# Lance0218/Pytorch-DistributedDataParallel-Training-Tricks

Measured on AMD Instinct MI355X. Metric: images/sec, higher is better.
Workload: dtype bf16; 1 GPU; model=Toy_Net, dataset=MNIST(synthetic), global_batch=1024, per_gpu_batch=1024, parallelism=dp1, optimizer=FusedSGD(momentum=0.9,nesterov)+Lookahead(k=10,a=0.5)

## Files before the change

### ddp_tricks_amd/ops/hip/bindings.cpp

```cpp
#include <torch/extension.h>

void multi_tensor_unscale(std::vector<at::Tensor> grads, at::Tensor found_inf,
                          double inv_scale,
                          c10::optional<at::Tensor> partials);
void multi_tensor_sqsum(std::vector<at::Tensor> tensors, at::Tensor partials);
void norm_finalize(at::Tensor partials, long n, double max_norm,
                   c10::optional<at::Tensor> found_inf, at::Tensor out,
                   c10::optional<at::Tensor> stats);
void multi_tensor_scale(std::vector<at::Tensor> tensors, at::Tensor coef,
                        c10::optional<at::Tensor> found_inf);
long mt_chunk_elems();
void fused_sgd(std::vector<at::Tensor> params, std::vector<at::Tensor> grads,
               std::vector<at::Tensor> bufs, double lr, double momentum,
               double wd, double nesterov, c10::optional<at::Tensor> found_inf,
               c10::optional<at::Tensor> grad_scale);
void fused_lookahead(std::vector<at::Tensor> fast, std::vector<at::Tensor> slow,
                     double alpha, c10::optional<at::Tensor> found_inf);
at::Tensor cast_to_bf16(at::Tensor x);
at::Tensor pad8_channels(at::Tensor x);
at::Tensor nhwc_flatten(at::Tensor x);
at::Tensor nhwc_unflatten(at::Tensor dy, long C, long H, long W);
std::vector<at::Tensor> pack_conv_weight(at::Tensor w, bool pad8,
                                         bool want_wt2);

std::vector<at::Tensor> ce_fwd(at::Tensor logits, at::Tensor target);
at::Tensor ce_bwd(at::Tensor logits, at::Tensor target, at::Tensor lse,
                  at::Tensor dloss);
at::Tensor argmax_correct(at::Tensor logits, at::Tensor target);

std::vector<at::Tensor> maxpool2x2_fwd(at::Tensor x);
at::Tensor maxpool2x2_bwd(at::Tensor dy, at::Tensor idx, long H, long W);
std::vector<at::Tensor> maxpool_fwd(at::Tensor x, long ks, long st, long pad);
at::Tensor maxpool_bwd(at::Tensor dy, at::Tensor idx, long H, long W,
                       long ks, long st, long pad);
at::Tensor global_avgpool_fwd(at::Tensor x);
at::Tensor global_avgpool_bwd(at::Tensor dy, long H, long W);

std::vector<at::Tensor> bn_fwd_train(at::Tensor x, at::Tensor gamma,
                                     at::Tensor beta, at::Tensor running_mean,
                                     at::Tensor running_var, double momentum,
                                     double eps, bool fuse_relu,
                                     c10::optional<at::Tensor> residual,
                                     c10::optional<at::Tensor> pre_stats);
at::Tensor bn_fwd_eval(at::Tensor x, at::Tensor gamma, at::Tensor beta,
                       at::Tensor running_mean, at::Tensor running_var,
                       double eps, bool fuse_relu,
                       c10::optional<at::Tensor> residual);
std::vector<at::Tensor> bn_fwd_eval_mask(at::Tensor x, at::Tensor gamma,
                                         at::Tensor beta,
                                         at::Tensor running_mean,
                                         at::Tensor running_var, double eps,
                                         bool fuse_relu,
                                         c10::optional<at::Tensor> residual);
std::vector<at::Tensor> bn_bwd(at::Tensor x, at::Tensor dy, at::Tensor gamma,
                               at::Tensor save_mean, at::Tensor save_invstd,
                               at::Tensor mask, bool fuse_relu,
                               bool want_dresid,
                               c10::optional<at::Tensor> pre_slab,
                               bool eval_stats);
std::vector<at::Tensor> bn_fwd_train_pool2(at::Tensor x, at::Tensor gamma,
                                           at::Tensor beta,
                                           at::Tensor running_mean,
                                           at::Tensor running_var,
                                           double momentum, double eps,
                                           c10::optional<at::Tensor> pre_stats);
std::vector<at::Tensor> bn_bwd_pool2(at::Tensor x, at::Tensor dy_pooled,
                                     at::Tensor gamma, at::Tensor save_mean,
                                     at::Tensor save_invstd, at::Tensor code);

at::Tensor gemm_tn(at::Tensor A, at::Tensor B, c10::optional<at::Tensor> bias,
                   bool out_f32);
at::Tensor transpose_bf16(at::Tensor x);
at::Tensor col_sum(at::Tensor x);
at::Tensor linear_fwd(at::Tensor x, at::Tensor w, c10::optional<at::Tensor> bias);
at::Tensor linear_dgrad(at::Tensor dy, at::Tensor w);
at::Tensor linear_wgrad(at::Tensor dy, at::Tensor x);

at::Tensor conv2d_fwd(at::Tensor x, at::Tensor w, c10::optional<at::Tensor> bias,
                      long stride, long pad);
std::vector<at::Tensor> conv2d_fwd_stats(at::Tensor x, at::Tensor w,
                                         c10::optional<at::Tensor> bias,
                                         long stride, long pad);
at::Tensor conv2d_dgrad(at::Tensor dy, at::Tensor wt2, long N, long C, long H,
                        long W, long R, long S, long stride, long pad,
                        c10::optional<at::Tensor> addend);
std::vector<at::Tensor> conv2d_dgrad_bn(at::Tensor dy, at::Tensor wt2,
                                        long N, long C, long H, long W,
                                        long R, long S, long pad,
                                        at::Tensor bn_x, at::Tensor bn_mask,
                                        at::Tensor bn_mean,
                                        at::Tensor bn_invstd);
at::Tensor conv2d_wgrad(at::Tensor dy, at::Tensor x, long R, long S,
                        long stride, long pad);
std::vector<at::Tensor> conv2d_wgrad_bias(at::Tensor dy, at::Tensor x,
                                          long R, long S, long stride,
                                          long pad);
std::tuple<std::string, long, bool> conv2d_wgrad_plan(
    long N, long C, long H, long W, long Ko, long R, long S, long stride,
    long pad, bool want_bias);

std::vector<at::Tensor> batch_gather_aug(at::Tensor store, at::Tensor labels,
                                         at::Tensor index, at::Tensor lut,
                                         long pad, bool hflip, long seed,
                                         long epoch);

void register_comm(py::module_& m);

PYBIND11_MODULE(TORCH_EXTENSION_NAME, m) {
    register_comm(m);
    m.def("multi_tensor_unscale", &multi_tensor_unscale,
          "fused unscale + inf check over grad tensors; with partials also "
          "the per-chunk sums of squares of the unscaled values",
          py::arg("grads"), py::arg("found_inf"), py::arg("inv_scale"),
          py::arg("partials") = c10::nullopt);
    m.def("multi_tensor_sqsum", &multi_tensor_sqsum,
          "per-chunk sums of squares (read-only)",
          py::arg("tensors"), py::arg("partials"));
    m.def("norm_finalize", &norm_finalize,
          "partials -> out = {2-norm, clip coefficient} (+ telemetry)",
          py::arg("partials"), py::arg("n"), py::arg("max_norm"),
          py::arg("found_inf"), py::arg("out"), py::arg("stats"));
    m.def("multi_tensor_scale", &multi_tensor_scale,
          "tensors *= coef[0] in place (device coefficient)",
          py::arg("tensors"), py::arg("coef"),
          py::arg("found_inf") = c10::nullopt);
    m.attr("MT_CHUNK") = mt_chunk_elems();
    m.def("fused_sgd", &fused_sgd, "fused nesterov-momentum SGD step",
          py::arg("params"), py::arg("grads"), py::arg("bufs"), py::arg("lr"),
          py::arg("momentum"), py::arg("wd"), py::arg("nesterov"),
          py::arg("found_inf") = c10::nullopt,
          py::arg("grad_scale") = c10::nullopt);
    m.def("fused_lookahead", &fused_lookahead, "fused Lookahead interpolation",
          py::arg("fast"), py::arg("slow"), py::arg("alpha"),
          py::arg("found_inf") = c10::nullopt);
    m.def("cast_to_bf16", &cast_to_bf16);
    m.def("pad8_channels", &pad8_channels);
    m.def("nhwc_flatten", &nhwc_flatten);
    m.def("nhwc_unflatten", &nhwc_unflatten);
    m.def("pack_conv_weight", &pack_conv_weight, py::arg("w"),
          py::arg("pad8") = false, py::arg("want_wt2") = true);
    m.def("ce_fwd", &ce_fwd);
    m.def("ce_bwd", &ce_bwd);
    m.def("argmax_correct", &argmax_correct);
    m.def("maxpool2x2_fwd", &maxpool2x2_fwd);
    m.def("maxpool2x2_bwd", &maxpool2x2_bwd);
    m.def("maxpool_fwd", &maxpool_fwd);
    m.def("maxpool_bwd", &maxpool_bwd);
    m.def("global_avgpool_fwd", &global_avgpool_fwd);
    m.def("global_avgpool_bwd", &global_avgpool_bwd);
    m.def("bn_fwd_train", &bn_fwd_train,
          py::arg("x"), py::arg("gamma"), py::arg("beta"),
          py::arg("running_mean"), py::arg("running_var"), py::arg("momentum"),
          py::arg("eps"), py::arg("fuse_relu") = false,
          py::arg("residual") = c10::nullopt,
          py::arg("pre_stats") = c10::nullopt);
    m.def("bn_fwd_eval", &bn_fwd_eval,
          py::arg("x"), py::arg("gamma"), py::arg("beta"),
          py::arg("running_mean"), py::arg("running_var"), py::arg("eps"),
          py::arg("fuse_relu") = false, py::arg("residual") = c10::nullopt);
    m.def("bn_bwd", &bn_bwd,
          py::arg("x"), py::arg("dy"), py::arg("gamma"), py::arg("save_mean"),
          py::arg("save_invstd"), py::arg("mask"), py::arg("fuse_relu") = false,
          py::arg("want_dresid") = false, py::arg("pre_slab") = c10::nullopt,
          py::arg("eval_stats") = false);
    m.def("bn_fwd_eval_mask", &bn_fwd_eval_mask,
          py::arg("x"), py::arg("gamma"), py::arg("beta"),
          py::arg("running_mean"), py::arg("running_var"), py::arg("eps"),
          py::arg("fuse_relu") = false, py::arg("residual") = c10::nullopt);
    m.def("bn_fwd_train_pool2", &bn_fwd_train_pool2,
          "BN(train) + ReLU + 2x2/s2 max-pool in one apply pass",
          py::arg("x"), py::arg("gamma"), py::arg("beta"),
          py::arg("running_mean"), py::arg("running_var"), py::arg("momentum"),
          py::arg("eps"), py::arg("pre_stats") = c10::nullopt);
    m.def("bn_bwd_pool2", &bn_bwd_pool2,
          py::arg("x"), py::arg("dy_pooled"), py::arg("gamma"),
          py::arg("save_mean"), py::arg("save_invstd"), py::arg("code"));
    m.def("gemm_tn", &gemm_tn, py::arg("A"), py::arg("B"),
          py::arg("bias") = c10::nullopt, py::arg("out_f32") = false);
    m.def("transpose_bf16", &transpose_bf16);
    m.def("col_sum", &col_sum);
    m.def("linear_fwd", &linear_fwd, py::arg("x"), py::arg("w"),
          py::arg("bias") = c10::nullopt);
    m.def("linear_dgrad", &linear_dgrad);
    m.def("linear_wgrad", &linear_wgrad);
    m.def("conv2d_fwd", &conv2d_fwd, py::arg("x"), py::arg("w"),
          py::arg("bias") = c10::nullopt, py::arg("stride") = 1,
          py::arg("pad") = 0);
    m.def("conv2d_fwd_stats", &conv2d_fwd_stats, py::arg("x"), py::arg("w"),
          py::arg("bias") = c10::nullopt, py::arg("stride") = 1,
          py::arg("pad") = 0);
    m.def("conv2d_dgrad", &conv2d_dgrad,
          py::arg("dy"), py::arg("wt2"), py::arg("N"), py::arg("C"),
          py::arg("H"), py::arg("W"), py::arg("R"), py::arg("S"),
          py::arg("stride"), py::arg("pad"),
          py::arg("addend") = c10::nullopt);
    m.def("conv2d_dgrad_bn", &conv2d_dgrad_bn);
    m.def("conv2d_wgrad", &conv2d_wgrad);
    m.def("conv2d_wgrad_bias", &conv2d_wgrad_bias);
    m.def("conv2d_wgrad_plan", &conv2d_wgrad_plan,
          "(leaf name, split, fused_bias) conv2d_wgrad[_bias] would run for "
          "this shape under this process's DDPX_WGRAD_V; launches nothing",
          py::arg("N"), py::arg("C"), py::arg("H"), py::arg("W"),
          py::arg("Ko"), py::arg("R"), py::arg("S"), py::arg("stride"),
          py::arg("pad"), py::arg("want_bias"));
    m.def("batch_gather_aug", &batch_gather_aug,
          "uint8 HWC device store -> (bf16 channels_last batch, labels): "
          "gather by index + crop/flip + LUT normalise in one launch",
          py::arg("store"), py::arg("labels"), py::arg("index"),
          py::arg("lut"), py::arg("pad"), py::arg("hflip"), py::arg("seed"),
          py::arg("epoch"));
}
```

### ddp_tricks_amd/ops/hip/conv.hip

```cpp

#include <torch/extension.h>
#include <ATen/hip/HIPContext.h>
#include <climits>
#include <string>
#include <tuple>
#include "common.h"

typedef short bf16x8_t __attribute__((ext_vector_type(8)));

constexpr int CBM = 128, CBK = 64;

struct ConvShape {
    int N, H, W, C;
    int Ko, R, S;
    int P, Q;
    int stride, pad;
    FastDiv fdQ, fdP, fdW, fdH, fdC, fdS, fdKo;
    int cls_a, cls_b, nr, ns;
    int taps_r[4], taps_s[4];
    int off_r[4], off_s[4];
    int Hfull, Wfull;
    FastDiv fdNs;
};

static inline void init_fastdiv(ConvShape& cs) {
    cs.fdQ.init(cs.Q); cs.fdP.init(cs.P); cs.fdW.init(cs.W);
    cs.fdH.init(cs.H); cs.fdC.init(cs.C); cs.fdS.init(cs.S);
    cs.fdKo.init(cs.Ko);
}


__device__ __align__(16) unsigned char g_zero16[16];

struct BnFuse {
    const bf16* x;
    const unsigned char* mask;
    const float* mean;
    const float* invstd;
    float* slab;
};

template <int MODE, int TBN, int WAVES_M, int WAVES_N, bool STRIDE1,
          int CBM_T>
__device__ __forceinline__
void conv_gemm_body(const bf16* __restrict__ Asrc,
                    const bf16* __restrict__ Bsrc,
                    const float* __restrict__ bias, bf16* __restrict__ out,
                    const ConvShape& cs, int M, int Kgemm, int Nout,
                    float* __restrict__ stats, BnFuse bn,
                    const bf16* __restrict__ addin) {
    constexpr int WM = CBM_T / WAVES_M;
    constexpr int WN = TBN / WAVES_N;
    constexpr int MI = WM / 16;
    constexpr int NI = WN / 16;
    constexpr int A_CHUNKS = CBM_T / 8;
    constexpr int B_CHUNKS = TBN / 8;
    __shared__ bf16 lds_a[1][CBM_T][CBK];
    __shared__ bf16 lds_b[1][TBN][CBK];
    const int m0 = blockIdx.x * CBM_T;
    const int n0 = blockIdx.y * TBN;
    const int tid = threadIdx.x;
    const int lane = tid & 63;
    const int wid = tid >> 6;
    const int wr = wid / WAVES_N, wc = wid % WAVES_N;

    f32x4 acc[MI][NI] = {};
    const int pl_row = lane >> 3;
    const int pl_segp = lane & 7;

    constexpr int A_PER = A_CHUNKS / 4;
    long ri_nb[A_PER];
    int ri_u[A_PER], ri_v[A_PER];
    #pragma unroll
    for (int ci = 0; ci < A_PER; ++ci) {
        const int ch = wid + ci * 4;
        const int row = ch * 8 + pl_row;
        const int gm = m0 + row;
        ri_u[ci] = INT_MIN;
        if (gm < M) {
            if (MODE == 0) {
                unsigned rem = fd_div(gm, cs.fdQ);
                int q = fd_mod(gm, cs.fdQ, rem);
                unsigned n = fd_div(rem, cs.fdP);
                int p = fd_mod(rem, cs.fdP, n);
                ri_nb[ci] = (long)n * cs.H;
                ri_u[ci] = p * cs.stride - cs.pad;
                ri_v[ci] = q * cs.stride - cs.pad;
            } else if (MODE == 2) {
                unsigned rem = fd_div(gm, cs.fdW);
                int w1 = fd_mod(gm, cs.fdW, rem);
                unsigned n = fd_div(rem, cs.fdH);
                int h1 = fd_mod(rem, cs.fdH, n);
                ri_nb[ci] = (long)n * cs.P;
                ri_u[ci] = h1;
                ri_v[ci] = w1;
            } else {
                unsigned rem = fd_div(gm, cs.fdW);
                int wcol = fd_mod(gm, cs.fdW, rem);
                unsigned n = fd_div(rem, cs.fdH);
                int h = fd_mod(rem, cs.fdH, n);
                ri_nb[ci] = (long)n * cs.P;
                ri_u[ci] = h + cs.pad;
                ri_v[ci] = wcol + cs.pad;
            }
        }
    }

    auto issue_tile = [&](int kt, int buf) {
        #pragma unroll
        for (int ci = 0; ci < A_PER; ++ci) {
            const int ch = wid + ci * 4;
            int row = ch * 8 + pl_row;
            int seg = pl_segp ^ (row & 7);
            int gk = kt + seg * 8;
            const bf16* src = reinterpret_cast<const bf16*>(g_zero16);
            if (ri_u[ci] != INT_MIN && gk < Kgemm) {
                if (MODE == 0) {
                    unsigned rs = fd_div(gk, cs.fdC);
                    int c = fd_mod(gk, cs.fdC, rs);
                    int r = fd_div(rs, cs.fdS);
                    int sx = fd_mod(rs, cs.fdS, r);
                    int h = ri_u[ci] + r;
                    int wcol = ri_v[ci] + sx;
                    if (h >= 0 && h < cs.H && wcol >= 0 && wcol < cs.W)
                        src = &Asrc[((ri_nb[ci] + h) * cs.W + wcol) * cs.C + c];
                } else if (MODE == 2) {
                    unsigned rs2 = fd_div(gk, cs.fdKo);
                    int ko = fd_mod(gk, cs.fdKo, rs2);
                    int ti = fd_div(rs2, cs.fdNs);
                    int si = fd_mod(rs2, cs.fdNs, ti);
                    int p = ri_u[ci] + cs.off_r[ti];
                    int q = ri_v[ci] + cs.off_s[si];
                    if (p >= 0 && p < cs.P && q >= 0 && q < cs.Q)
                        src = &Asrc[((ri_nb[ci] + p) * cs.Q + q) * cs.Ko + ko];
                } else if (STRIDE1) {
                    unsigned rs = fd_div(gk, cs.fdKo);
                    int ko = fd_mod(gk, cs.fdKo, rs);
                    int r = fd_div(rs, cs.fdS);
                    int sx = fd_mod(rs, cs.fdS, r);
                    int p = ri_u[ci] - r;
                    int q = ri_v[ci] - sx;
                    if (p >= 0 && p < cs.P && q >= 0 && q < cs.Q)
                        src = &Asrc[((ri_nb[ci] + p) * cs.Q + q) * cs.Ko + ko];
                } else {
                    unsigned rs = fd_div(gk, cs.fdKo);
                    int ko = fd_mod(gk, cs.fdKo, rs);
                    int r = fd_div(rs, cs.fdS);
                    int sx = fd_mod(rs, cs.fdS, r);
                    int pn = ri_u[ci] - r;
                    int qn = ri_v[ci] - sx;
                    int p = pn / cs.stride, q = qn / cs.stride;
                    if (pn >= 0 && qn >= 0 && pn == p * cs.stride &&
                        qn == q * cs.stride && p < cs.P && q < cs.Q)
                        src = &Asrc[((ri_nb[ci] + p) * cs.Q + q) * cs.Ko + ko];
                }
            }
            __builtin_amdgcn_global_load_lds(
                (const __attribute__((address_space(1))) unsigned short*)src,
                (__attribute__((address_space(3))) unsigned short*)&lds_a[buf][ch * 8][0],
                16, 0, 0);
        }
        for (int ch = wid; ch < B_CHUNKS; ch += 4) {
            int row = ch * 8 + pl_row;
            int seg = pl_segp ^ (row & 7);
            int gn = n0 + row, gk = kt + seg * 8;
            const bf16* src = reinterpret_cast<const bf16*>(g_zero16);
            if (MODE == 2) {
                if (gn < Nout && gk < Kgemm) {
                    unsigned rs2 = fd_div(gk, cs.fdKo);
                    int ko = fd_mod(gk, cs.fdKo, rs2);
                    int ri = fd_div(rs2, cs.fdNs);
                    int si = fd_mod(rs2, cs.fdNs, ri);
                    long gk_full = ((long)cs.taps_r[ri] * cs.S
                                    + cs.taps_s[si]) * cs.Ko + ko;
                    src = &Bsrc[(long)gn * (cs.R * cs.S * cs.Ko) + gk_full];
                }
            } else if (gn < Nout && gk < Kgemm)
                src = &Bsrc[(long)gn * Kgemm + gk];
            __builtin_amdgcn_global_load_lds(
                (const __attribute__((address_space(1))) unsigned short*)src,
                (__attribute__((address_space(3))) unsigned short*)&lds_b[buf][ch * 8][0],
                16, 0, 0);
        }
    };

    constexpr int buf = 0;
    for (int kt = 0; kt < Kgemm; kt += CBK) {
        issue_tile(kt, 0);
        __syncthreads();
        #pragma unroll
        for (int ks = 0; ks < CBK; ks += 32) {
            bf16x8_t af[MI], bfr[NI];
            const int kgrp = (ks >> 3) + (lane >> 4);
            #pragma unroll
            for (int mi = 0; mi < MI; ++mi) {
                int row = wr * WM + mi * 16 + (lane & 15);
                af[mi] = *reinterpret_cast<const bf16x8_t*>(
                    &lds_a[buf][row][(kgrp ^ (row & 7)) * 8]);
            }
            #pragma unroll
            for (int ni = 0; ni < NI; ++ni) {
                int row = wc * WN + ni * 16 + (lane & 15);
                bfr[ni] = *reinterpret_cast<const bf16x8_t*>(
                    &lds_b[buf][row][(kgrp ^ (row & 7)) * 8]);
            }
            #pragma unroll
            for (int mi = 0; mi < MI; ++mi)
                #pragma unroll
                for (int ni = 0; ni < NI; ++ni)
                    acc[mi][ni] = __builtin_amdgcn_mfma_f32_16x16x32_bf16(
                        af[mi], bfr[ni], acc[mi][ni], 0, 0, 0);
        }
        __syncthreads();
    }

    float psum[NI] = {}, psq[NI] = {};
    #pragma unroll
    for (int mi = 0; mi < MI; ++mi)
        #pragma unroll
        for (int ni = 0; ni < NI; ++ni) {
            int col = n0 + wc * WN + ni * 16 + (lane & 15);
            if (col >= Nout) continue;
            float badd = bias ? bias[col] : 0.f;
            #pragma unroll
            for (int r = 0; r < 4; ++r) {
                int row = m0 + wr * WM + mi * 16 + (lane >> 4) * 4 + r;
                if (row >= M) continue;
                if (MODE == 0 && stats) {
                    float v = acc[mi][ni][r] + badd;
                    psum[ni] += v;
                    psq[ni] = fmaf(v, v, psq[ni]);
                }
                if (MODE == 2) {
                    unsigned rem = fd_div(row, cs.fdW);
                    int w1 = fd_mod(row, cs.fdW, rem);
                    unsigned n = fd_div(rem, cs.fdH);
                    int h1 = fd_mod(rem, cs.fdH, n);
                    long addr = (((long)n * cs.Hfull + cs.cls_a
                                  + (long)h1 * cs.stride) * cs.Wfull
                                 + cs.cls_b + (long)w1 * cs.stride) * Nout
                                + col;
                    out[addr] = f2bf(acc[mi][ni][r] + badd);
                }
            }
        }

    if (MODE != 2) {
        __syncthreads();
        bf16* stageA = &lds_a[0][0][0];
        bf16* stageB = &lds_b[0][0][0];
        constexpr int HALF = CBM_T * CBK;
        auto stage_at = [&](int i) -> bf16& {
            return i < HALF ? stageA[i] : stageB[i - HALF];
        };
        #pragma unroll
        for (int mi = 0; mi < MI; ++mi)
            #pragma unroll
            for (int ni = 0; ni < NI; ++ni) {
                int cl = wc * WN + ni * 16 + (lane & 15);
                float badd2 = (bias && n0 + cl < Nout) ? bias[n0 + cl] : 0.f;
                #pragma unroll
                for (int r = 0; r < 4; ++r) {
                    int rl = wr * WM + mi * 16 + (lane >> 4) * 4 + r;
                    stage_at(rl * TBN + cl) = f2bf(acc[mi][ni][r] + badd2);
                }
            }
        __syncthreads();
        constexpr int ROWS_PER_PASS = 256 / (TBN / 8);
        const int rsub = tid / (TBN / 8);
        const int csub = (tid % (TBN / 8)) * 8;
        const bool do_bn = MODE == 1 && bn.slab != nullptr;
        float bsum[8] = {}, bsx[8] = {};
        float bmean[8], binv[8];
        if (do_bn && n0 + csub < Nout) {
            #pragma unroll
            for (int j = 0; j < 8; ++j) {
                bmean[j] = bn.mean[n0 + csub + j];
                binv[j] = bn.invstd[n0 + csub + j];
            }
        }
        for (int r0_ = 0; r0_ < CBM_T; r0_ += ROWS_PER_PASS) {
            int rl = r0_ + rsub;
            long row = (long)m0 + rl;
            int col = n0 + csub;
            if (rl < CBM_T && row < M && col < Nout) {
                int i = rl * TBN + csub;
                const bf16* src16 = i < HALF ? &stageA[i] : &stageB[i - HALF];
                bf16x8_t v = *reinterpret_cast<const bf16x8_t*>(src16);
                if (MODE == 1 && addin) {
                    s16x8 a8 = *reinterpret_cast<const s16x8*>(
                        &addin[row * Nout + col]);
                    s16x8& vv = reinterpret_cast<s16x8&>(v);
                    #pragma unroll
                    for (int j = 0; j < 8; ++j)
                        vv[j] = (short)f2us(us2f((unsigned short)vv[j])
                                            + us2f((unsigned short)a8[j]));
                }
                *reinterpret_cast<bf16x8_t*>(&out[row * Nout + col]) = v;
                if (do_bn) {
                    unsigned m8 = bn.mask
                        ? bn.mask[row * (Nout >> 3) + (col >> 3)] : 0xffu;
                    s16x8 xv = *reinterpret_cast<const s16x8*>(
                        &bn.x[row * Nout + col]);
                    #pragma unroll
                    for (int j = 0; j < 8; ++j) {
                        float g = (m8 >> j) & 1u
                            ? us2f((unsigned short)((s16x8&)v)[j]) : 0.f;
                        float xh = (us2f((unsigned short)xv[j]) - bmean[j])
                                   * binv[j];
                        bsum[j] += g;
                        bsx[j] = fmaf(g, xh, bsx[j]);
                    }
                }
            }
        }
        if (do_bn) {
            __syncthreads();
            float* red = reinterpret_cast<float*>(stageA);
            #pragma unroll
            for (int j = 0; j < 8; ++j) {
                red[(rsub * TBN + csub + j) * 2] = bsum[j];
                red[(rsub * TBN + csub + j) * 2 + 1] = bsx[j];
            }
            __syncthreads();
            const int gridM = gridDim.x;
            for (int cl = tid; cl < TBN; cl += 256) {
                float a = 0.f, b2 = 0.f;
                #pragma unroll 4
                for (int w = 0; w < ROWS_PER_PASS; ++w) {
                    a += red[(w * TBN + cl) * 2];
                    b2 += red[(w * TBN + cl) * 2 + 1];
                }
                int col = n0 + cl;
                if (col < Nout) {
                    bn.slab[(long)col * gridM + blockIdx.x] = a;
                    bn.slab[(long)Nout * gridM + (long)col * gridM
                            + blockIdx.x] = b2;
                }
            }
        }
    }

    if (MODE == 0 && stats) {
        __syncthreads();
        float* red = reinterpret_cast<float*>(&lds_a[0][0][0]);
        #pragma unroll
        for (int ni = 0; ni < NI; ++ni) {
            float a = psum[ni], b = psq[ni];
            a += __shfl_down(a, 32, 64);
            a += __shfl_down(a, 16, 64);
            b += __shfl_down(b, 32, 64);
            b += __shfl_down(b, 16, 64);
            if ((lane & 48) == 0) {
                int cl = wc * WN + ni * 16 + (lane & 15);
                red[(wr * TBN + cl) * 2] = a;
                red[(wr * TBN + cl) * 2 + 1] = b;
            }
        }
        __syncthreads();
        const int gridM = gridDim.x;
        for (int cl = tid; cl < TBN; cl += 256) {
            float a = 0.f, b = 0.f;
            #pragma unroll
            for (int w = 0; w < WAVES_M; ++w) {
                a += red[(w * TBN + cl) * 2];
                b += red[(w * TBN + cl) * 2 + 1];
            }
            int col = n0 + cl;
            if (col < Nout) {
                stats[(long)col * gridM + blockIdx.x] = a;
                stats[(long)Nout * gridM + (long)col * gridM + blockIdx.x] = b;
            }
        }
    }
}

template <int MODE, int TBN, int WAVES_M, int WAVES_N, bool STRIDE1 = true,
          int CBM_T = CBM>
__global__ __launch_bounds__(256, 4)
void k_conv_gemm(const bf16* __restrict__ Asrc, const bf16* __restrict__ Bsrc,
                 const float* __restrict__ bias, bf16* __restrict__ out,
                 ConvShape cs, int M, int Kgemm, int Nout,
                 float* __restrict__ stats = nullptr,
                 BnFuse bn = BnFuse{},
                 const bf16* __restrict__ addin = nullptr) {
    conv_gemm_body<MODE, TBN, WAVES_M, WAVES_N, STRIDE1, CBM_T>(
        Asrc, Bsrc, bias, out, cs, M, Kgemm, Nout, stats, bn, addin);
}


struct ClsPack {
    ConvShape cs[4];
    int M[4];
    int K[4];
};

template <int TBN, int WAVES_M, int WAVES_N>
__global__ __launch_bounds__(256, 4)
void k_conv_gemm_cls(const bf16* __restrict__ Asrc,
                     const bf16* __restrict__ Bsrc, bf16* __restrict__ out,
                     ClsPack pack, int Nout) {
    const int z = blockIdx.z;
    const int M = pack.M[z];
    if ((int)blockIdx.x * CBM >= M) return;
    conv_gemm_body<2, TBN, WAVES_M, WAVES_N, true, CBM>(
        Asrc, Bsrc, nullptr, out, pack.cs[z], M, pack.K[z], Nout,
        nullptr, BnFuse{}, nullptr);
}

__global__ void k_conv_small_cin(const bf16* __restrict__ x,
                                 const bf16* __restrict__ w,
                                 const float* __restrict__ bias,
                                 bf16* __restrict__ y, ConvShape cs, long M) {
    extern __shared__ __attribute__((aligned(16))) char smem[];
    bf16* wlds = reinterpret_cast<bf16*>(smem);
    int rsc = cs.R * cs.S * cs.C;
    for (int i = threadIdx.x; i < cs.Ko * rsc; i += blockDim.x)
        wlds[i] = w[i];
    __syncthreads();
    long total = M * (cs.Ko / 8);
    long i = (long)blockIdx.x * blockDim.x + threadIdx.x;
    long gstride = (long)gridDim.x * blockDim.x;
    for (; i < total; i += gstride) {
        int ko8 = (i % (cs.Ko / 8)) * 8;
        long gm = i / (cs.Ko / 8);
        int q = gm % cs.Q; long rem = gm / cs.Q;
        int p = rem % cs.P; int n = rem / cs.P;
        float acc[8] = {};
        for (int r = 0; r < cs.R; ++r) {
            int h = p * cs.stride + r - cs.pad;
            if (h < 0 || h >= cs.H) continue;
            for (int s = 0; s < cs.S; ++s) {
                int wc = q * cs.stride + s - cs.pad;
                if (wc < 0 || wc >= cs.W) continue;
                for (int c = 0; c < cs.C; ++c) {
                    float xv = bf2f(x[(((long)n * cs.H + h) * cs.W + wc) * cs.C + c]);
                    int kidx = (r * cs.S + s) * cs.C + c;
                    #pragma unroll
                    for (int j = 0; j < 8; ++j)
                        acc[j] = fmaf(xv, bf2f(wlds[(ko8 + j) * rsc + kidx]), acc[j]);
                }
            }
        }
        bf16x8_t o;
        #pragma unroll
        for (int j = 0; j < 8; ++j)
            o[j] = (short)f2us(acc[j] + (bias ? bias[ko8 + j] : 0.f));
        *reinterpret_cast<bf16x8_t*>(&y[gm * cs.Ko + ko8]) = o;
    }
}


constexpr int WBM = 64, WBN = 64;

template <bool BIAS = false>
__global__ void k_wgrad_combine(const float* __restrict__ slab, int S,
                                ConvShape cs, int Kgemm,
                                float* __restrict__ dw,
                                float* __restrict__ db) {
    long total = (long)cs.Ko * Kgemm;
    const int nb = BIAS ? gridDim.x - 1 : gridDim.x;
    if (BIAS && (int)blockIdx.x == nb) {
        const float* bs = slab + (long)S * total;
        for (int ko = threadIdx.x; ko < cs.Ko; ko += blockDim.x) {
            float v = 0.f;
            for (int s = 0; s < S; ++s) v += bs[(long)s * cs.Ko + ko];
            db[ko] = v;
        }
        return;
    }
    long i = (long)blockIdx.x * blockDim.x + threadIdx.x;
    long stride = (long)nb * blockDim.x;
    int RS = cs.R * cs.S;
    for (; i < total; i += stride) {
        float v = 0.f;
        for (int s = 0; s < S; ++s) v += slab[(long)s * total + i];
        int ko = i / Kgemm;
        int rc = i % Kgemm;
        int c = rc % cs.C, rs = rc / cs.C;
        dw[((long)ko * cs.C + c) * RS + rs] = v;
    }
}

template <bool BIAS = false>
__global__ void k_wgrad_combine_stage(const float* __restrict__ slab, int S,
                                      int CH, long total, int Ko,
                                      float* __restrict__ slab2) {
    long i = (long)blockIdx.x * blockDim.x + threadIdx.x;
    if (i >= (BIAS ? total + Ko : total)) return;
    const int c0 = blockIdx.y * CH;
    const int ce = min(S, c0 + CH);
    long ld = total;
    if (BIAS && i >= total) {
        slab += (long)S * total - total;
        slab2 += (long)gridDim.y * total - total;
        ld = Ko;
    }
    float v0 = 0.f, v1 = 0.f;
    int s = c0;
    for (; s + 1 < ce; s += 2) {
        v0 += slab[(long)s * ld + i];
        v1 += slab[(long)(s + 1) * ld + i];
    }
    if (s < ce) v0 += slab[(long)s * ld + i];
    slab2[(long)blockIdx.y * ld + i] = v0 + v1;
}

template <int DEPTH>
__global__ __launch_bounds__(256)
void k_conv_wgrad_sb_pair(const bf16* __restrict__ dy,
                          const bf16* __restrict__ x,
                          float* __restrict__ slab, ConvShape cs, long M,
                          int Kgemm, int S) {
    __shared__ bf16 lds_a[WBM][DEPTH + 8];
    __shared__ bf16 lds_b[WBN][DEPTH + 8];
    constexpr int SLD = DEPTH + 8;
    constexpr int PAIRS = DEPTH / 2;
    const int ko0 = blockIdx.x * WBM;
    const int rc0 = blockIdx.y * WBN;
    const int split = blockIdx.z;
    const int tid = threadIdx.x;
    const int lane = tid & 63;
    const int wid = tid >> 6, wr = wid >> 1, wc = wid & 1;

    f32x4 acc[2][2] = {};
    const int m2 = (tid & (PAIRS - 1)) * 2;
    const int jsel = tid / PAIRS;
    constexpr int JSLOTS = 256 / PAIRS;
    const bool is_b = jsel >= JSLOTS / 2;
    const int jb = (jsel % (JSLOTS / 2)) * 8;
    constexpr int JSTEP = (JSLOTS / 2) * 8;

    const long m_begin = (long)split * DEPTH;
    for (long mt = m_begin; mt < M; mt += (long)S * DEPTH) {
        long gm0 = mt + m2;
        const bool v0 = gm0 < M, v1 = gm0 + 1 < M;
        unsigned q0 = 0, p0 = 0, n0_ = 0, q1 = 0, p1 = 0, n1_ = 0;
        if (is_b) {
            if (v0) {
// ... 642 lines not shown
            acc = fmaf(bf2f(dy[gm * cs.Ko + ko]), xv, acc);
        }
    }
    red[walker][kl] = acc;
    __syncthreads();
    if (walker == 0 && ko < cs.Ko) {
        float t = 0.f;
        #pragma unroll
        for (int w = 0; w < 4; ++w) t += red[w][kl];
        slab[((long)split * gridDim.x + rsc) * cs.Ko + ko] = t;
    }
}

__global__ void k_wgrad_small_combine(const float* __restrict__ slab, int S,
                                      ConvShape cs, int rsc_total,
                                      float* __restrict__ dw) {
    int i = blockIdx.x * blockDim.x + threadIdx.x;
    if (i >= rsc_total * cs.Ko) return;
    int ko = i % cs.Ko;
    int rc = i / cs.Ko;
    float v = 0.f;
    for (int s = 0; s < S; ++s)
        v += slab[((long)s * rsc_total + rc) * cs.Ko + ko];
    int c = rc % cs.C, rs = rc / cs.C;
    dw[((long)ko * cs.C + c) * (cs.R * cs.S) + rs] = v;
}


static ConvShape make_shape(int N, int C, int H, int W, int Ko, int R, int S,
                            int stride, int pad) {
    ConvShape cs;
    cs.N = N; cs.C = C; cs.H = H; cs.W = W;
    cs.Ko = Ko; cs.R = R; cs.S = S; cs.stride = stride; cs.pad = pad;
    cs.P = (cs.H + 2 * pad - R) / stride + 1;
    cs.Q = (cs.W + 2 * pad - S) / stride + 1;
    init_fastdiv(cs);
    return cs;
}

static ConvShape make_shape(const at::Tensor& x, int Ko, int R, int S,
                            int stride, int pad) {
    return make_shape(x.size(0), x.size(1), x.size(2), x.size(3), Ko, R, S,
                      stride, pad);
}

static at::Tensor empty_nhwc(const at::Tensor& like, long n, long c, long h,
                             long w) {
    return at::empty({n, c, h, w},
                     like.options().memory_format(at::MemoryFormat::ChannelsLast));
}

template <int MODE, bool STRIDE1 = true>
static void launch_conv_gemm(hipStream_t stream, int grid_m, int n_channels,
                             bool narrow, const bf16* Asrc, const bf16* Bsrc,
                             const float* bias, bf16* out,
                             const ConvShape& cs, long M, int Kgemm,
                             float* stats, BnFuse bn, const bf16* addin) {
    if (n_channels >= 128 && !narrow)
        hipLaunchKernelGGL((k_conv_gemm<MODE, 128, 2, 2, STRIDE1>),
                           dim3(grid_m, ceil_div_i(n_channels, 128)),
                           dim3(256), 0, stream, Asrc, Bsrc, bias, out, cs,
                           (int)M, Kgemm, n_channels, stats, bn, addin);
    else
        hipLaunchKernelGGL((k_conv_gemm<MODE, 64, 4, 1, STRIDE1>),
                           dim3(grid_m, ceil_div_i(n_channels, 64)),
                           dim3(256), 0, stream, Asrc, Bsrc, bias, out, cs,
                           (int)M, Kgemm, n_channels, stats, bn, addin);
    HIP_CHECK_LAST();
}

static void launch_conv_gemm_cls(hipStream_t stream, int grid_m,
                                 int n_channels, int ncls, const bf16* Asrc,
                                 const bf16* Bsrc, bf16* out,
                                 const ClsPack& pack) {
    if (n_channels >= 128)
        hipLaunchKernelGGL((k_conv_gemm_cls<128, 2, 2>),
                           dim3(grid_m, ceil_div_i(n_channels, 128), ncls),
                           dim3(256), 0, stream, Asrc, Bsrc, out, pack,
                           n_channels);
    else
        hipLaunchKernelGGL((k_conv_gemm_cls<64, 4, 1>),
                           dim3(grid_m, ceil_div_i(n_channels, 64), ncls),
                           dim3(256), 0, stream, Asrc, Bsrc, out, pack,
                           n_channels);
    HIP_CHECK_LAST();
}

static std::vector<at::Tensor> conv_fwd_impl(
        const at::Tensor& x, const at::Tensor& w,
        const c10::optional<at::Tensor>& bias, long stride, long pad,
        bool want_stats) {
    TORCH_CHECK(x.is_cuda() && x.scalar_type() == at::kBFloat16);
    ConvShape cs = make_shape(x, w.size(0), w.size(2), w.size(3),
                              (int)stride, (int)pad);
    int Kgemm = cs.R * cs.S * cs.C;
    long M = (long)cs.N * cs.P * cs.Q;
    auto stream = at::hip::getCurrentHIPStream();
    const float* bp = bias.has_value() ? bias->data_ptr<float>() : nullptr;
    const bf16* xp = reinterpret_cast<const bf16*>(x.data_ptr());
    const bf16* wp = reinterpret_cast<const bf16*>(w.data_ptr());
    auto y = empty_nhwc(x, cs.N, cs.Ko, cs.P, cs.Q);
    bf16* yp = reinterpret_cast<bf16*>(y.data_ptr());

    if (cs.C < 8 && !want_stats) {
        TORCH_CHECK(cs.Ko % 8 == 0);
        int lds = cs.Ko * Kgemm * 2;
        long total = M * (cs.Ko / 8);
        int blocks = std::min<long>(8192, ceil_div_i(total, 256));
        hipLaunchKernelGGL(k_conv_small_cin, dim3(blocks), dim3(256), lds,
                           stream.stream(), xp, wp, bp, yp, cs, M);
        HIP_CHECK_LAST();
        return {y, at::Tensor()};
    }
    TORCH_CHECK(cs.C % 8 == 0, want_stats
                ? "stats path needs the MFMA conv (C%8==0)"
                : "conv fwd needs C % 8 == 0");
    TORCH_CHECK(cs.Ko % 8 == 0, "conv fwd needs Ko % 8 == 0");
    const int gridM = ceil_div_i(M, CBM);
    at::Tensor slab;
    if (want_stats)
        slab = at::empty({2, (long)cs.Ko, (long)gridM},
                         x.options().dtype(at::kFloat));
    static const char* tbn_env = getenv("DDPX_CONV_TBN64");
    launch_conv_gemm<0>(stream.stream(), gridM, cs.Ko,
                        tbn_env && !want_stats, xp, wp, bp, yp, cs, M, Kgemm,
                        want_stats ? slab.data_ptr<float>() : nullptr,
                        BnFuse{}, nullptr);
    return {y, slab};
}

at::Tensor conv2d_fwd(at::Tensor x, at::Tensor w,
                      c10::optional<at::Tensor> bias, long stride, long pad) {
    return conv_fwd_impl(x, w, bias, stride, pad, false)[0];
}

std::vector<at::Tensor> conv2d_fwd_stats(at::Tensor x, at::Tensor w,
                                         c10::optional<at::Tensor> bias,
                                         long stride, long pad) {
    return conv_fwd_impl(x, w, bias, stride, pad, true);
}

static ConvShape dgrad_shape(const at::Tensor& dy, long N, long C, long H,
                             long W, long R, long S, long stride, long pad) {
    ConvShape cs;
    cs.N = N; cs.C = C; cs.H = H; cs.W = W;
    cs.Ko = dy.size(1); cs.P = dy.size(2); cs.Q = dy.size(3);
    cs.R = R; cs.S = S; cs.stride = stride; cs.pad = pad;
    init_fastdiv(cs);
    TORCH_CHECK(cs.Ko % 8 == 0, "conv dgrad needs Ko % 8 == 0");
    TORCH_CHECK(cs.C % 8 == 0, "conv dgrad needs C % 8 == 0");
    return cs;
}

static at::Tensor dgrad_stride1(const at::Tensor& dy, const at::Tensor& wt2,
                                const ConvShape& cs,
                                const c10::optional<at::Tensor>& addend,
                                BnFuse bn) {
    auto dx = empty_nhwc(dy, cs.N, cs.C, cs.H, cs.W);
    const bf16* adp = nullptr;
    if (addend.has_value()) {
        TORCH_CHECK(addend->sizes() == dx.sizes() &&
                    addend->scalar_type() == at::kBFloat16);
        adp = reinterpret_cast<const bf16*>(addend->data_ptr());
    }
    const long M = (long)cs.N * cs.H * cs.W;
    launch_conv_gemm<1>(at::hip::getCurrentHIPStream().stream(),
                        ceil_div_i(M, CBM), cs.C, false,
                        reinterpret_cast<const bf16*>(dy.data_ptr()),
                        reinterpret_cast<const bf16*>(wt2.data_ptr()),
                        nullptr, reinterpret_cast<bf16*>(dx.data_ptr()), cs,
                        M, cs.R * cs.S * cs.Ko, nullptr, bn, adp);
    return dx;
}

at::Tensor conv2d_dgrad(at::Tensor dy, at::Tensor wt2, long N, long C,
                        long H, long W, long R, long S, long stride, long pad,
                        c10::optional<at::Tensor> addend) {
    ConvShape cs = dgrad_shape(dy, N, C, H, W, R, S, stride, pad);
    TORCH_CHECK(!addend.has_value() || cs.stride == 1,
                "fused dgrad addend needs stride 1");
    if (cs.stride == 1) return dgrad_stride1(dy, wt2, cs, addend, BnFuse{});

    auto dx = empty_nhwc(dy, cs.N, cs.C, cs.H, cs.W);
    auto stream = at::hip::getCurrentHIPStream();
    const bf16* dyp_ = reinterpret_cast<const bf16*>(dy.data_ptr());
    const bf16* wt2p = reinterpret_cast<const bf16*>(wt2.data_ptr());
    bf16* dxp = reinterpret_cast<bf16*>(dx.data_ptr());
    const int st = cs.stride;
    {
        bool any_empty = false;
        for (int a = 0; a < st && !any_empty; ++a) {
            int nr = 0;
            for (int r = 0; r < cs.R; ++r)
                if (((a + cs.pad - r) % st + st) % st == 0) ++nr;
            if (nr == 0) any_empty = true;
        }
        if (!any_empty)
            for (int b = 0; b < st && !any_empty; ++b) {
                int ns = 0;
                for (int sidx = 0; sidx < cs.S; ++sidx)
                    if (((b + cs.pad - sidx) % st + st) % st == 0) ++ns;
                if (ns == 0) any_empty = true;
            }
        if (any_empty) dx.zero_();
    }
    ClsPack pack{};
    int ncls = 0;
    int maxTiles = 0;
    for (int a = 0; a < st; ++a) {
        for (int b = 0; b < st; ++b) {
            ConvShape c2 = cs;
            c2.cls_a = a; c2.cls_b = b;
            c2.Hfull = cs.H; c2.Wfull = cs.W;
            c2.nr = 0; c2.ns = 0;
            for (int r = 0; r < cs.R; ++r)
                if (((a + cs.pad - r) % st + st) % st == 0) {
                    c2.taps_r[c2.nr] = r;
                    c2.off_r[c2.nr] = (a + cs.pad - r) / st;
                    ++c2.nr;
                }
            for (int sidx = 0; sidx < cs.S; ++sidx)
                if (((b + cs.pad - sidx) % st + st) % st == 0) {
                    c2.taps_s[c2.ns] = sidx;
                    c2.off_s[c2.ns] = (b + cs.pad - sidx) / st;
                    ++c2.ns;
                }
            if (c2.nr == 0 || c2.ns == 0) continue;
            int Ha = (cs.H - a + st - 1) / st;
            int Wb = (cs.W - b + st - 1) / st;
            c2.H = Ha; c2.W = Wb;
            c2.fdH.init(Ha); c2.fdW.init(Wb);
            c2.fdNs.init(c2.ns);
            long M2 = (long)cs.N * Ha * Wb;
            int K2 = c2.nr * c2.ns * cs.Ko;
            if (ncls < 4) {
                pack.cs[ncls] = c2;
                pack.M[ncls] = (int)M2;
                pack.K[ncls] = K2;
                maxTiles = std::max(maxTiles, (int)ceil_div_i(M2, CBM));
                ++ncls;
            } else {
                launch_conv_gemm<2>(stream.stream(), ceil_div_i(M2, CBM),
                                    cs.C, false, dyp_, wt2p, nullptr, dxp,
                                    c2, M2, K2, nullptr, BnFuse{}, nullptr);
            }
        }
    }
    if (ncls > 0)
        launch_conv_gemm_cls(stream.stream(), maxTiles, cs.C, ncls, dyp_,
                             wt2p, dxp, pack);
    return dx;
}

std::vector<at::Tensor> conv2d_dgrad_bn(at::Tensor dy, at::Tensor wt2,
                                        long N, long C, long H, long W,
                                        long R, long S, long pad,
                                        at::Tensor bn_x, at::Tensor bn_mask,
                                        at::Tensor bn_mean,
                                        at::Tensor bn_invstd) {
    ConvShape cs = dgrad_shape(dy, N, C, H, W, R, S, 1, pad);
    const int gridM = ceil_div_i((long)cs.N * cs.H * cs.W, CBM);
    auto slab = at::empty({2, (long)cs.C, (long)gridM},
                          dy.options().dtype(at::kFloat));
    BnFuse bn;
    bn.x = reinterpret_cast<const bf16*>(bn_x.data_ptr());
    bn.mask = bn_mask.numel()
        ? bn_mask.data_ptr<unsigned char>() : nullptr;
    bn.mean = bn_mean.data_ptr<float>();
    bn.invstd = bn_invstd.data_ptr<float>();
    bn.slab = slab.data_ptr<float>();
    return {dgrad_stride1(dy, wt2, cs, c10::nullopt, bn), slab};
}

at::Tensor col_sum(at::Tensor x);


enum class WgradLeaf {
    StemStream, C1R3, SmallRsc, SmallCin,
    SbPair32, SbPair64,
    WidePair32, WidePair64, WideDma32, WideDma64,
};

using WgradMfmaKernel = void (*)(const bf16*, const bf16*, float*, ConvShape,
                                 long, int, int);
static const struct { const char* name; WgradMfmaKernel kern[2]; }
WGRAD_LEAVES[] = {
    {"c1_r3_stream", {}}, {"c1_r3", {}}, {"small_rsc", {}}, {"small_cin", {}},
    {"sb_pair<32>", {k_conv_wgrad_sb_pair<32>, k_conv_wgrad_sb_pair<32>}},
    {"sb_pair<64>", {k_conv_wgrad_sb_pair<64>, k_conv_wgrad_sb_pair<64>}},
    {"wide_pair<32>", {k_conv_wgrad_wide_pair<32, false>,
                       k_conv_wgrad_wide_pair<32, true>}},
    {"wide_pair<64>", {k_conv_wgrad_wide_pair<64, false>,
                       k_conv_wgrad_wide_pair<64, true>}},
    {"wide_dma<32>", {k_conv_wgrad_wide_dma<32, false>,
                      k_conv_wgrad_wide_dma<32, true>}},
    {"wide_dma<64>", {k_conv_wgrad_wide_dma<64, false>,
                      k_conv_wgrad_wide_dma<64, true>}},
};
static_assert(sizeof(WGRAD_LEAVES) / sizeof(WGRAD_LEAVES[0]) ==
              (int)WgradLeaf::WideDma64 + 1, "one row per WgradLeaf");

struct WgradPlan {
    WgradLeaf leaf;
    int S;
    int gk, gr;
    bool fused_bias;
};

static const char* wgrad_override() {
    static const char* v = getenv("DDPX_WGRAD_V");
    return v;
}

static WgradPlan plan_wgrad(const ConvShape& cs, long M, bool want_bias,
                            const char* override) {
    enum { Auto, Dma, Dma32, Pair64, Pair32, Sb32, Sb64 } force = Auto;
    if (override && override[0]) {
        const std::string v(override);
        if (v == "wt") force = Dma;
        else if (v == "wt3") force = Dma32;
        else if (v == "wp") force = Pair64;
        else if (v == "wq") force = Pair32;
        else if (v == "s" || v == "sb") force = Sb32;
        else if (v == "s6") force = Sb64;
        else TORCH_CHECK(false, "DDPX_WGRAD_V=", v, " selects no wgrad "
                         "kernel; accepted values: wt, wt3, wp, wq, s, sb, "
                         "s6 (unset or empty: automatic)");
    }
    const int Kgemm = cs.R * cs.S * cs.C;
    WgradPlan p{};

    if (cs.C < 8) {
        const bool c1r3 = cs.C == 1 && cs.R == 3 && cs.S == 3;
        if (c1r3 && cs.Ko % 8 == 0 && cs.Ko <= 64 && M < INT_MAX) {
            const int rpl = 64 / (cs.Ko / 8);
            const long nloads = (M + rpl - 1) / rpl;
            p.leaf = WgradLeaf::StemStream;
            p.S = (int)std::max<long>(
                1, std::min<long>(768, (nloads + 8 * SU - 1) / (8 * SU)));
            p.fused_bias = want_bias;
        } else if (Kgemm <= 16 && cs.Ko <= 64) {
            p.leaf = c1r3 ? WgradLeaf::C1R3 : WgradLeaf::SmallRsc;
            p.S = (int)std::max<long>(1, std::min<long>(2048, M / 8));
        } else {
            p.leaf = WgradLeaf::SmallCin;
            p.S = 64;
        }
        return p;
    }

    TORCH_CHECK(cs.C % 8 == 0 && cs.Ko % 8 == 0);
    const bool can_wide = cs.Ko >= 128 && Kgemm >= 128;
    const bool enough = can_wide &&
        (ceil_div_i(cs.Ko, 128) * ceil_div_i(Kgemm, 128) >= 8
         || M >= 262144);
    const bool wide = force == Auto
        ? enough
        : can_wide && force != Sb32 && force != Sb64;
    const int tile = wide ? 128 : WBM;
    p.gk = ceil_div_i(cs.Ko, tile);
    p.gr = ceil_div_i(Kgemm, tile);
    if (wide) {
        const bool deep = Kgemm >= 1152;
        p.leaf = force == Pair64 ? WgradLeaf::WidePair64
               : force == Pair32 ? WgradLeaf::WidePair32
               : force == Dma32 || !deep ? WgradLeaf::WideDma32
               : WgradLeaf::WideDma64;
    } else {
        const bool sb64 = force == Auto ? p.gk == 1 && p.gr <= 8
                                        : force == Sb64;
        p.leaf = sb64 ? WgradLeaf::SbPair64 : WgradLeaf::SbPair32;
    }
    const int count_depth = wide ? 64 : 32;
    p.S = 1;
    while (p.gk * p.gr * p.S < 1024 && p.S < 512 &&
           M / ((long)p.S * 2 * count_depth) >= 8) p.S *= 2;
    p.fused_bias = want_bias && wide;
    return p;
}

std::tuple<std::string, long, bool> conv2d_wgrad_plan(
        long N, long C, long H, long W, long Ko, long R, long S, long stride,
        long pad, bool want_bias) {
    TORCH_CHECK(N > 0 && C > 0 && Ko > 0 && R > 0 && S > 0 && stride > 0 &&
                pad >= 0 && H + 2 * pad >= R && W + 2 * pad >= S);
    ConvShape cs = make_shape((int)N, (int)C, (int)H, (int)W, (int)Ko, (int)R,
                              (int)S, (int)stride, (int)pad);
    WgradPlan p = plan_wgrad(cs, (long)cs.N * cs.P * cs.Q, want_bias,
                             wgrad_override());
    return std::make_tuple(std::string(WGRAD_LEAVES[(int)p.leaf].name),
                           (long)p.S, p.fused_bias);
}

static std::vector<at::Tensor> wgrad_impl(const at::Tensor& dy,
                                          const at::Tensor& x, long R,
                                          long S, long stride, long pad,
                                          bool want_bias) {
    ConvShape cs = make_shape(x, dy.size(1), (int)R, (int)S, (int)stride,
                              (int)pad);
    TORCH_CHECK(cs.P == dy.size(2) && cs.Q == dy.size(3));
    const long M = (long)cs.N * cs.P * cs.Q;
    const int Kgemm = cs.R * cs.S * cs.C;
    const WgradPlan plan = plan_wgrad(cs, M, want_bias, wgrad_override());
    const int S_ = plan.S;
    const bool fused_bias = plan.fused_bias;

    auto stream = at::hip::getCurrentHIPStream();
    const auto f32 = x.options().dtype(at::kFloat);
    auto dw = at::empty({(long)cs.Ko, (long)cs.C, (long)cs.R, (long)cs.S},
                        f32);
    at::Tensor db;
    if (fused_bias) db = at::empty({(long)cs.Ko}, f32);
    float* dbp = fused_bias ? db.data_ptr<float>() : nullptr;
    const bf16* dyp = reinterpret_cast<const bf16*>(dy.data_ptr());
    const bf16* xp = reinterpret_cast<const bf16*>(x.data_ptr());

    switch (plan.leaf) {
    case WgradLeaf::StemStream:
    case WgradLeaf::C1R3:
    case WgradLeaf::SmallRsc: {
        const int nt = Kgemm + fused_bias;
        auto slab = at::empty({nt * cs.Ko, S_}, f32);
        if (plan.leaf == WgradLeaf::StemStream) {
            const int rpl = 64 / (cs.Ko / 8);
// ... 90 lines not shown
```

Measured before the change: 385,500 images/sec.

## Skip zero-contribution filter taps in stride-1 conv dgrad via grouped M raster

Adds a tap-uniform M ordering for stride-1 dgrad with no padding. Rows are grouped so each 128-row tile covers the same spatial pixels across G images, which lets the kernel compute a per-tile mask of filter taps that fall inside the output and skip K tiles for the rest. Output rows are remapped back to NHWC on store, and block indices are swizzled across groups of eight. The path is chosen automatically only for two hard-coded layer shapes at N>=1024, and the extra index arithmetic and changed access locality could offset the skipped MFMA work.

```diff
diff --git a/ddp_tricks_amd/ops/hip/bindings.cpp b/ddp_tricks_amd/ops/hip/bindings.cpp
--- a/ddp_tricks_amd/ops/hip/bindings.cpp
+++ b/ddp_tricks_amd/ops/hip/bindings.cpp
@@ -83,7 +83,10 @@
                                          long stride, long pad);
 at::Tensor conv2d_dgrad(at::Tensor dy, at::Tensor wt2, long N, long C, long H,
                         long W, long R, long S, long stride, long pad,
-                        c10::optional<at::Tensor> addend);
+                        c10::optional<at::Tensor> addend, long group);
+std::tuple<std::string, long, long, long> conv2d_dgrad_plan(
+    long N, long C, long H, long W, long Ko, long R, long S, long stride,
+    long pad, long group);
 std::vector<at::Tensor> conv2d_dgrad_bn(at::Tensor dy, at::Tensor wt2,
                                         long N, long C, long H, long W,
                                         long R, long S, long pad,
@@ -193,7 +196,14 @@
           py::arg("dy"), py::arg("wt2"), py::arg("N"), py::arg("C"),
           py::arg("H"), py::arg("W"), py::arg("R"), py::arg("S"),
           py::arg("stride"), py::arg("pad"),
-          py::arg("addend") = c10::nullopt);
+          py::arg("addend") = c10::nullopt, py::arg("group") = -1);
+    m.def("conv2d_dgrad_plan", &conv2d_dgrad_plan,
+          "(name, G, k_tiles_issued, k_tiles_raster) conv2d_dgrad would run "
+          "for this shape; group -1 automatic, 0 raster, 32/64/128 forces "
+          "that tap-uniform group size; launches nothing",
+          py::arg("N"), py::arg("C"), py::arg("H"), py::arg("W"),
+          py::arg("Ko"), py::arg("R"), py::arg("S"), py::arg("stride"),
+          py::arg("pad"), py::arg("group") = -1);
     m.def("conv2d_dgrad_bn", &conv2d_dgrad_bn);
     m.def("conv2d_wgrad", &conv2d_wgrad);
     m.def("conv2d_wgrad_bias", &conv2d_wgrad_bias);
diff --git a/ddp_tricks_amd/ops/hip/conv.hip b/ddp_tricks_amd/ops/hip/conv.hip
--- a/ddp_tricks_amd/ops/hip/conv.hip
+++ b/ddp_tricks_amd/ops/hip/conv.hip
@@ -21,12 +21,40 @@
     int off_r[4], off_s[4];
     int Hfull, Wfull;
     FastDiv fdNs;
+    FastDiv fdGHW;
+    int lgG;
 };
 
 static inline void init_fastdiv(ConvShape& cs) {
     cs.fdQ.init(cs.Q); cs.fdP.init(cs.P); cs.fdW.init(cs.W);
     cs.fdH.init(cs.H); cs.fdC.init(cs.C); cs.fdS.init(cs.S);
     cs.fdKo.init(cs.Ko);
+    cs.fdGHW.init(1); cs.lgG = 0;
+}
+
+__host__ __device__ inline unsigned dgrad_tap_mask(
+        int m_first, int m_last, int GHW, int lgG, int H, int W, int P, int Q,
+        int R, int S, int pad) {
+    const int g0 = m_first / GHW, g1 = m_last / GHW;
+    int pix0 = 0, pix1 = H * W - 1;
+    if (g0 == g1) {
+        pix0 = (m_first - g0 * GHW) >> lgG;
+        pix1 = (m_last - g0 * GHW) >> lgG;
+    }
+    const int h0 = pix0 / W, h1 = pix1 / W;
+    unsigned mask = 0;
+    for (int h = h0; h <= h1; ++h) {
+        const int wa = h == h0 ? pix0 - h0 * W : 0;
+        const int wb = h == h1 ? pix1 - h1 * W : W - 1;
+        const int ra = h + pad - P + 1 > 0 ? h + pad - P + 1 : 0;
+        const int rb = h + pad < R - 1 ? h + pad : R - 1;
+        const int sa = wa + pad - Q + 1 > 0 ? wa + pad - Q + 1 : 0;
+        const int sb = wb + pad < S - 1 ? wb + pad : S - 1;
+        for (int r = ra; r <= rb; ++r)
+            for (int sx = sa; sx <= sb; ++sx)
+                mask |= 1u << (r * S + sx);
+    }
+    return mask;
 }
 
 
@@ -41,7 +69,7 @@
 };
 
 template <int MODE, int TBN, int WAVES_M, int WAVES_N, bool STRIDE1,
-          int CBM_T>
+          int CBM_T, bool TAPS = false>
 __device__ __forceinline__
 void conv_gemm_body(const bf16* __restrict__ Asrc,
                     const bf16* __restrict__ Bsrc,
@@ -57,7 +85,11 @@
     constexpr int B_CHUNKS = TBN / 8;
     __shared__ bf16 lds_a[1][CBM_T][CBK];
     __shared__ bf16 lds_b[1][TBN][CBK];
-    const int m0 = blockIdx.x * CBM_T;
+    static_assert(!TAPS || (MODE == 1 && STRIDE1), "TAPS is stride-1 dgrad");
+    const int tile_m = TAPS && (gridDim.x & 7) == 0
+        ? (int)(blockIdx.x & 7) * (int)(gridDim.x >> 3) + (int)(blockIdx.x >> 3)
+        : (int)blockIdx.x;
+    const int m0 = tile_m * CBM_T;
     const int n0 = blockIdx.y * TBN;
     const int tid = threadIdx.x;
     const int lane = tid & 63;
@@ -94,6 +126,16 @@
                 ri_nb[ci] = (long)n * cs.P;
                 ri_u[ci] = h1;
                 ri_v[ci] = w1;
+            } else if (TAPS) {
+                unsigned grp = fd_div(gm, cs.fdGHW);
+                unsigned rem = fd_mod(gm, cs.fdGHW, grp);
+                unsigned pix = rem >> cs.lgG;
+                unsigned n = (grp << cs.lgG) + (rem & ((1u << cs.lgG) - 1));
+                unsigned h = fd_div(pix, cs.fdW);
+                int wcol = fd_mod(pix, cs.fdW, h);
+                ri_nb[ci] = (long)n * cs.P;
+                ri_u[ci] = (int)h + cs.pad;
+                ri_v[ci] = wcol + cs.pad;
             } else {
                 unsigned rem = fd_div(gm, cs.fdW);
                 int wcol = fd_mod(gm, cs.fdW, rem);
@@ -185,7 +227,17 @@
     };
 
     constexpr int buf = 0;
+    unsigned tap_mask = 0;
+    if (TAPS)
+        tap_mask = __builtin_amdgcn_readfirstlane(dgrad_tap_mask(
+            m0, min(m0 + CBM_T, M) - 1, (int)cs.fdGHW.d, cs.lgG, cs.H, cs.W,
+            cs.P, cs.Q, cs.R, cs.S, cs.pad));
+    int tap = 0, tap_end = cs.Ko;
     for (int kt = 0; kt < Kgemm; kt += CBK) {
+        if (TAPS) {
+            if (kt == tap_end) { ++tap; tap_end += cs.Ko; }
+            if (!((tap_mask >> tap) & 1u)) { kt = tap_end - CBK; continue; }
+        }
         issue_tile(kt, 0);
         __syncthreads();
         #pragma unroll
@@ -283,7 +335,15 @@
             int rl = r0_ + rsub;
             long row = (long)m0 + rl;
             int col = n0 + csub;
-            if (rl < CBM_T && row < M && col < Nout) {
+            const bool live = rl < CBM_T && row < M && col < Nout;
+            if (TAPS && live) {
+                unsigned gm = (unsigned)row;
+                unsigned grp = fd_div(gm, cs.fdGHW);
+                unsigned rem = fd_mod(gm, cs.fdGHW, grp);
+                unsigned n = (grp << cs.lgG) + (rem & ((1u << cs.lgG) - 1));
+                row = (long)n * (cs.H * cs.W) + (rem >> cs.lgG);
+            }
+            if (live) {
                 int i = rl * TBN + csub;
                 const bf16* src16 = i < HALF ? &stageA[i] : &stageB[i - HALF];
                 bf16x8_t v = *reinterpret_cast<const bf16x8_t*>(src16);
@@ -376,7 +436,7 @@
 }
 
 template <int MODE, int TBN, int WAVES_M, int WAVES_N, bool STRIDE1 = true,
-          int CBM_T = CBM>
+          int CBM_T = CBM, bool TAPS = false>
 __global__ __launch_bounds__(256, 4)
 void k_conv_gemm(const bf16* __restrict__ Asrc, const bf16* __restrict__ Bsrc,
                  const float* __restrict__ bias, bf16* __restrict__ out,
@@ -384,7 +444,7 @@
                  float* __restrict__ stats = nullptr,
                  BnFuse bn = BnFuse{},
                  const bf16* __restrict__ addin = nullptr) {
-    conv_gemm_body<MODE, TBN, WAVES_M, WAVES_N, STRIDE1, CBM_T>(
+    conv_gemm_body<MODE, TBN, WAVES_M, WAVES_N, STRIDE1, CBM_T, TAPS>(
         Asrc, Bsrc, bias, out, cs, M, Kgemm, Nout, stats, bn, addin);
 }
 
@@ -1333,10 +1393,65 @@
     return cs;
 }
 
+struct DgradPlan {
+    const char* name;
+    int G;
+    long k_tiles, k_tiles_raster;
+};
+
+static DgradPlan plan_dgrad(const ConvShape& cs, bool want_bn, long group) {
+    TORCH_CHECK(group == -1 || group == 0 || group == 32 || group == 64 ||
+                group == 128, "conv dgrad group must be -1 (automatic), 0 "
+                "(raster), 32, 64 or 128; got ", group);
+    const long M = (long)cs.N * cs.H * cs.W;
+    const int tiles = ceil_div_i(M, CBM);
+    DgradPlan p{"raster", 0, 0, 0};
+    p.k_tiles_raster = (long)tiles * ceil_div_i((long)cs.R * cs.S * cs.Ko, CBK);
+    p.k_tiles = p.k_tiles_raster;
+    const bool fits = cs.stride == 1 && cs.Ko % CBK == 0 &&
+                      cs.R * cs.S <= 32 && !want_bn && M < INT_MAX;
+    if (!fits || group == 0) return p;
+
+    auto count = [&](int G) {
+        int lg = 0;
+        while ((1 << lg) < G) ++lg;
+        const long ghw = (long)G * cs.H * cs.W;
+        const bool periodic = ghw % CBM == 0;
+        const int walk = periodic ? (int)(ghw / CBM) : tiles;
+        long n = 0;
+        for (int t = 0; t < walk; ++t) {
+            const int m0 = t * CBM;
+            const int m1 = (int)std::min<long>(m0 + CBM, M) - 1;
+            n += __builtin_popcount(dgrad_tap_mask(
+                m0, m1, (int)ghw, lg, cs.H, cs.W, cs.P, cs.Q, cs.R, cs.S,
+                cs.pad));
+        }
+        if (periodic) n *= cs.N / G;
+        return n * (cs.Ko / CBK);
+    };
+    static const struct { int C, H, W, Ko, R, S, pad, G; } MEASURED[] = {
+        {128, 12, 12, 256, 3, 3, 0, 128},
+        {256, 10, 10, 512, 3, 3, 0, 128},
+    };
+    int G = (int)std::max<long>(group, 0);
+    if (group < 0 && cs.N >= 1024)
+        for (const auto& m : MEASURED)
+            if (cs.C == m.C && cs.H == m.H && cs.W == m.W && cs.Ko == m.Ko &&
+                cs.R == m.R && cs.S == m.S && cs.pad == m.pad)
+                G = m.G;
+    if (G == 0 || cs.N % G != 0) return p;
+    const long issued = count(G);
+    if (issued >= p.k_tiles_raster) return p;
+    p.name = "taps";
+    p.G = G;
+    p.k_tiles = issued;
+    return p;
+}
+
 static at::Tensor dgrad_stride1(const at::Tensor& dy, const at::Tensor& wt2,
-                                const ConvShape& cs,
+                                ConvShape cs,
                                 const c10::optional<at::Tensor>& addend,
-                                BnFuse bn) {
+                                BnFuse bn, long group) {
     auto dx = empty_nhwc(dy, cs.N, cs.C, cs.H, cs.W);
     const bf16* adp = nullptr;
     if (addend.has_value()) {
@@ -1345,22 +1460,44 @@
         adp = reinterpret_cast<const bf16*>(addend->data_ptr());
     }
     const long M = (long)cs.N * cs.H * cs.W;
-    launch_conv_gemm<1>(at::hip::getCurrentHIPStream().stream(),
-                        ceil_div_i(M, CBM), cs.C, false,
-                        reinterpret_cast<const bf16*>(dy.data_ptr()),
-                        reinterpret_cast<const bf16*>(wt2.data_ptr()),
-                        nullptr, reinterpret_cast<bf16*>(dx.data_ptr()), cs,
-                        M, cs.R * cs.S * cs.Ko, nullptr, bn, adp);
+    const int grid_m = ceil_div_i(M, CBM);
+    const int Kgemm = cs.R * cs.S * cs.Ko;
+    auto stream = at::hip::getCurrentHIPStream().stream();
+    const bf16* dyp = reinterpret_cast<const bf16*>(dy.data_ptr());
+    const bf16* wtp = reinterpret_cast<const bf16*>(wt2.data_ptr());
+    bf16* dxp = reinterpret_cast<bf16*>(dx.data_ptr());
+    const DgradPlan plan = plan_dgrad(cs, bn.slab != nullptr, group);
+    if (plan.G == 0) {
+        launch_conv_gemm<1>(stream, grid_m, cs.C, false, dyp, wtp, nullptr,
+                            dxp, cs, M, Kgemm, nullptr, bn, adp);
+        return dx;
+    }
+    cs.fdGHW.init((unsigned)plan.G * cs.H * cs.W);
+    cs.lgG = 0;
+    while ((1 << cs.lgG) < plan.G) ++cs.lgG;
+    if (cs.C >= 128)
+        hipLaunchKernelGGL((k_conv_gemm<1, 128, 2, 2, true, CBM, true>),
+                           dim3(grid_m, ceil_div_i(cs.C, 128)), dim3(256), 0,
+                           stream, dyp, wtp, nullptr, dxp, cs, (int)M, Kgemm,
+                           cs.C, nullptr, BnFuse{}, adp);
+    else
+        hipLaunchKernelGGL((k_conv_gemm<1, 64, 4, 1, true, CBM, true>),
+                           dim3(grid_m, ceil_div_i(cs.C, 64)), dim3(256), 0,
+                           stream, dyp, wtp, nullptr, dxp, cs, (int)M, Kgemm,
+                           cs.C, nullptr, BnFuse{}, adp);
+    HIP_CHECK_LAST();
     return dx;
 }
 
 at::Tensor conv2d_dgrad(at::Tensor dy, at::Tensor wt2, long N, long C,
                         long H, long W, long R, long S, long stride, long pad,
-                        c10::optional<at::Tensor> addend) {
+                        c10::optional<at::Tensor> addend, long group) {
     ConvShape cs = dgrad_shape(dy, N, C, H, W, R, S, stride, pad);
     TORCH_CHECK(!addend.has_value() || cs.stride == 1,
                 "fused dgrad addend needs stride 1");
-    if (cs.stride == 1) return dgrad_stride1(dy, wt2, cs, addend, BnFuse{});
+    if (cs.stride == 1)
+        return dgrad_stride1(dy, wt2, cs, addend, BnFuse{}, group);
+    plan_dgrad(cs, false, group);
 
     auto dx = empty_nhwc(dy, cs.N, cs.C, cs.H, cs.W);
     auto stream = at::hip::getCurrentHIPStream();
@@ -1450,7 +1587,19 @@
     bn.mean = bn_mean.data_ptr<float>();
     bn.invstd = bn_invstd.data_ptr<float>();
     bn.slab = slab.data_ptr<float>();
-    return {dgrad_stride1(dy, wt2, cs, c10::nullopt, bn), slab};
+    return {dgrad_stride1(dy, wt2, cs, c10::nullopt, bn, -1), slab};
+}
+
+std::tuple<std::string, long, long, long> conv2d_dgrad_plan(
+        long N, long C, long H, long W, long Ko, long R, long S, long stride,
+        long pad, long group) {
+    TORCH_CHECK(N > 0 && C > 0 && Ko > 0 && R > 0 && S > 0 && stride > 0 &&
+                pad >= 0 && H + 2 * pad >= R && W + 2 * pad >= S);
+    ConvShape cs = make_shape((int)N, (int)C, (int)H, (int)W, (int)Ko, (int)R,
+                              (int)S, (int)stride, (int)pad);
+    const DgradPlan p = plan_dgrad(cs, false, group);
+    return std::make_tuple(std::string(p.name), (long)p.G, p.k_tiles,
+                           p.k_tiles_raster);
 }
 
 at::Tensor col_sum(at::Tensor x);
```

After: 404,000 images/sec (median of 6 runs). +4.8%, better.
